# KohakuBlueleaf/UwUDiff

Measured on AMD Instinct MI355X. Metric: train images/sec (whole node), DiT-S/2 256^2 latent, higher is better.
Workload: dtype bf16; 1 GPU; DiT-S/2 (L12 D384 h6), 4x32x32 synthetic latents + pooled-text cond 1280, eps-MSE, AdamW lr1e-6 wd0.01 cosine; random-init weights; per_gpu_batch=768, global_batch=768, parallelism=dp1

## Files before the change

uwudiff_amd/csrc/attention_p256.hip:

```cpp
#include "common.h"

namespace {

constexpr int P_RING = 3;
template <int DH>
struct PGeom {
  static constexpr bool TAIL = DH > 64;
  static constexpr int SLOT = 16384 + (TAIL ? 2048 + 256 : 0);
  static constexpr int OFF_TT = 16384, OFF_TL = 16384 + 2048;
  static constexpr int OFF_DS = P_RING * SLOT;
  static constexpr int KIMG = 32768 + (TAIL ? 4096 : 0);
  static constexpr int OFF_K = OFF_DS + 32768;
  static constexpr int OFF_LSE = OFF_K + 2 * KIMG;
  static constexpr int OFF_DELTA = OFF_LSE + (TAIL ? 0 : 2 * 1024);
  static constexpr int OFF_ZERO = OFF_DELTA + 2 * 256;
  static constexpr int LDS = OFF_ZERO + (TAIL ? 16 : 0);
};
static_assert(PGeom<64>::LDS == 150016 && PGeom<72>::LDS <= 163840, "LDS budget");
constexpr int P_LDS = PGeom<64>::LDS;

struct PArgs {
  const bf16_t *q, *k, *v, *o, *dO;
  bf16_t *dq, *dk, *dv;
  const float* lse;
  int B, H, ldq, ldk, ldv, ldo, nheads;
  float scale;
};

__device__ __forceinline__ int fsw(int row) {
  return (((row >> 2) ^ (row >> 4)) & 1) | ((((row >> 3) ^ (row >> 4)) & 1) << 1) | (((row >> 1) & 1) << 2);
}
__device__ __forceinline__ int Fsw(int row) {
  return (row & 1) | (((row >> 2) & 1) << 1) | (((row >> 3) & 1) << 2) | (((row >> 1) & 1) << 3);
}

typedef short s16x4 __attribute__((ext_vector_type(4)));
typedef unsigned su32x2 __attribute__((ext_vector_type(2)));

__device__ __forceinline__ void glds16(const void* gsrc, unsigned lds_dst ) {
  unsigned keep;
  asm volatile("s_mov_b32 %0, m0\n\ts_mov_b32 m0, %2\n\ts_nop 0\n\tglobal_load_lds_dwordx4 %1, off\n\ts_mov_b32 m0, %0"
               : "=&s"(keep)
               : "v"(gsrc), "s"(lds_dst)
               : "memory");
}
__device__ __forceinline__ void glds4(const void* gsrc, unsigned lds_dst ) {
  unsigned keep;
  asm volatile("s_mov_b32 %0, m0\n\ts_mov_b32 m0, %2\n\ts_nop 0\n\tglobal_load_lds_dword %1, off\n\ts_mov_b32 m0, %0"
               : "=&s"(keep)
               : "v"(gsrc), "s"(lds_dst)
               : "memory");
}
__device__ __forceinline__ void glds16_s(const void* sbase , unsigned voff, unsigned lds_dst ) {
  unsigned keep;
  asm volatile("s_mov_b32 %0, m0\n\ts_mov_b32 m0, %3\n\ts_nop 0\n\tglobal_load_lds_dwordx4 %1, %2\n\ts_mov_b32 m0, %0"
               : "=&s"(keep)
               : "v"(voff), "s"(sbase), "s"(lds_dst)
               : "memory");
}
__device__ __forceinline__ f32x16 mfma32(const uint4& a, const uint4& b, f32x16 c) {
  return __builtin_amdgcn_mfma_f32_32x32x16_bf16(*reinterpret_cast<const bf16x8*>(&a), *reinterpret_cast<const bf16x8*>(&b), c, 0,
                                                 0, 0);
}
__device__ __forceinline__ f32x4 mfma16(const uint4& a, const uint4& b, f32x4 c) {
  return __builtin_amdgcn_mfma_f32_16x16x32_bf16(*reinterpret_cast<const bf16x8*>(&a), *reinterpret_cast<const bf16x8*>(&b), c, 0,
                                                 0, 0);
}
__device__ __forceinline__ uint4 pack8(const f32x16& x, int s) {
  bf16x8 f;
#pragma unroll
  for (int j = 0; j < 8; ++j) f[j] = (bf16_t)x[8 * s + j];
  return *reinterpret_cast<uint4*>(&f);
}

extern __shared__ __attribute__((aligned(16))) char p_smem[];

__device__ __forceinline__ void lane_halves(float x, float& lo, float& hi) {
  float a = x, b = x;
  asm volatile("v_nop\n\tv_nop\n\tv_permlane32_swap_b32 %0, %1" : "+v"(a), "+v"(b));
  lo = a;
  hi = b;
}

__device__ __forceinline__ uint4 tr_pair(unsigned a0, unsigned a1) {
  const s16x4 lo = __builtin_amdgcn_ds_read_tr16_b64_v4i16(
      (__attribute__((address_space(3))) s16x4*)((__attribute__((address_space(3))) char*)p_smem + a0));
  const s16x4 hi = __builtin_amdgcn_ds_read_tr16_b64_v4i16(
      (__attribute__((address_space(3))) s16x4*)((__attribute__((address_space(3))) char*)p_smem + a1));
  uint4 r;
  r.x = ((unsigned)(unsigned short)lo[0]) | ((unsigned)(unsigned short)lo[1] << 16);
  r.y = ((unsigned)(unsigned short)lo[2]) | ((unsigned)(unsigned short)lo[3] << 16);
  r.z = ((unsigned)(unsigned short)hi[0]) | ((unsigned)(unsigned short)hi[1] << 16);
  r.w = ((unsigned)(unsigned short)hi[2]) | ((unsigned)(unsigned short)hi[3] << 16);
  return r;
}

template <int DH>
__global__ void __launch_bounds__(512, 2) attn_bwd_p256(const PArgs a) {
  using G = PGeom<DH>;
  constexpr bool TAIL = G::TAIL;
  constexpr int T = 256, NKS = TAIL ? 5 : 4, NDT = TAIL ? 3 : 2;
  constexpr int P_SLOT = G::SLOT, P_OFF_DS = G::OFF_DS, P_OFF_K = G::OFF_K, P_OFF_LSE = G::OFF_LSE, P_OFF_DELTA = G::OFF_DELTA;
  constexpr int KIMG = G::KIMG;
  char* const smem = p_smem;
  const int tid = threadIdx.x, lane = tid & 63;
  const int wave = __builtin_amdgcn_readfirstlane(tid >> 6);
  const int r = lane & 31, h = lane >> 5;
  const int fr = lane & 15, fq = lane >> 4;
  const unsigned smem_base = (unsigned)(size_t)((const __attribute__((address_space(3))) char*)p_smem);
  const float c = a.scale * 1.4426950408889634f;
  const float ninv_scale = -1.f / a.scale;
  const int nmy = (a.nheads - (int)blockIdx.x + (int)gridDim.x - 1) / (int)gridDim.x;
  const int total = 4 * nmy;
  const int k0 = wave * 32;

  const int drow = tid >> 3;
  const int dchunk = (tid & 7) ^ fsw(drow);
  unsigned B0, A0, K0, D0, TQ0, TA0, KT0;
  auto phase1_consts = [&](int ln) {
    const int r_ = ln & 31, h_ = ln >> 5;
    B0 = (unsigned)(r_ * 128 + ((h_ ^ fsw(r_)) << 4));
    const int rowL = 4 * h_ + ((ln & 15) >> 2), chunkL = 2 * ((ln >> 4) & 1) + ((ln & 3) >> 1);
    A0 = (unsigned)(rowL * 128 + ((chunkL ^ fsw(rowL)) << 4) + 8 * (ln & 1));
    TQ0 = (unsigned)((r_ >> 3) * 256 + (r_ & 7) * 16);
    TA0 = (unsigned)(rowL * 16 + 8 * (ln & 1));
  };
  auto phase2_consts = [&](int ln) {
    const int fr_ = ln & 15, fq_ = ln >> 4;
    const int rowK = 8 * fq_ + (fr_ >> 2);
    K0 = (unsigned)(rowK * 128 + ((((fr_ & 3) >> 1) ^ fsw(rowK)) << 4) + 8 * (fr_ & 1));
    D0 = (unsigned)(rowK * 128 + (((fr_ & 3) ^ Fsw(rowK)) << 3));
    KT0 = (unsigned)(rowK * 16 + 8 * (fr_ & 1));
  };
  auto opaque_lane = [&]() {
    int ln = lane;
    asm volatile("" : "+v"(ln));
    return ln;
  };
  auto my_tid = [&]() {
    int x = tid;
    if constexpr (TAIL) asm volatile("" : "+v"(x));
    return x;
  };
  if constexpr (!TAIL) {
    phase1_consts(lane);
    phase2_consts(lane);
  }

  auto head_ptrs = [&](int j, int& b, int& hd) {
    const int bh = (int)blockIdx.x + j * (int)gridDim.x;
    b = bh / a.H;
    hd = bh - b * a.H;
  };
  uint4 oreg;
  unsigned otail = 0;
  auto issue_tile = [&](int g) {
    int b, hd;
    head_ptrs(g >> 2, b, hd);
    const int tid = my_tid(), lane = tid & 63, drow = tid >> 3, dchunk = (tid & 7) ^ fsw(drow);
    const int row = 64 * (g & 3) + drow;
    const bf16_t* qs = a.q + ((int64_t)b * T + row) * a.ldq + hd * DH + 8 * dchunk;
    const bf16_t* gs = a.dO + ((int64_t)b * T + row) * a.ldo + hd * DH + 8 * dchunk;
    const unsigned dst = smem_base + (unsigned)((g % P_RING) * P_SLOT + wave * 1024);
    glds16(qs, dst);
    glds16(gs, dst + 8192);
    oreg = *reinterpret_cast<const uint4*>(a.o + ((int64_t)b * T + row) * a.ldo + hd * DH + 8 * dchunk);
    if constexpr (TAIL) {
      const unsigned slot = smem_base + (unsigned)((g % P_RING) * P_SLOT);
      if (lane < 16) {
        const int64_t trow = (int64_t)b * T + 64 * (g & 3) + 8 * wave + (lane & 7);
        const bf16_t* src = lane < 8 ? a.q + trow * a.ldq + hd * DH + 64 : a.dO + trow * a.ldo + hd * DH + 64;
        glds16(src, slot + (unsigned)(G::OFF_TT + wave * 256));
      }
      glds4(a.lse + ((int64_t)b * a.H + hd) * T + 64 * (g & 3) + lane, slot + (unsigned)G::OFF_TL);
      otail = *reinterpret_cast<const unsigned*>(a.o + ((int64_t)b * T + row) * a.ldo + hd * DH + 64 + 2 * (tid & 3));
    }
  };
  auto issue_head = [&](int j) {
    int b, hd;
    head_ptrs(j, b, hd);
    const int tid = my_tid(), lane = tid & 63, drow = tid >> 3, dchunk = (tid & 7) ^ fsw(drow);
    const unsigned dst = smem_base + (unsigned)(P_OFF_K + (j & 1) * KIMG + wave * 1024);
#pragma unroll
    for (int p = 0; p < 4; ++p)
      glds16(a.k + ((int64_t)b * T + 64 * p + drow) * a.ldk + hd * DH + 8 * dchunk, dst + p * 8192);
    if constexpr (TAIL) {
      if (lane < 32)
        glds16(a.k + ((int64_t)b * T + 32 * wave + lane) * a.ldk + hd * DH + 64,
               smem_base + (unsigned)(P_OFF_K + (j & 1) * KIMG + 32768 + wave * 512));
    } else {
      glds4(a.lse + ((int64_t)b * a.H + hd) * T + 64 * (wave & 3) + lane,
            smem_base + (unsigned)(P_OFF_LSE + (j & 1) * 1024 + (wave & 3) * 256));
    }
  };
  uint4 kf[NKS], vf[NKS];
  auto load_kv = [&](int j) {
    int b, hd;
    head_ptrs(j, b, hd);
    const int tid = my_tid(), r = tid & 31, h = (tid >> 5) & 1;
#pragma unroll
    for (int s = 0; s < 4; ++s) {
      kf[s] = *reinterpret_cast<const uint4*>(a.k + ((int64_t)b * T + k0 + r) * a.ldk + hd * DH + 16 * s + 8 * h);
      vf[s] = *reinterpret_cast<const uint4*>(a.v + ((int64_t)b * T + k0 + r) * a.ldv + hd * DH + 16 * s + 8 * h);
    }
    if constexpr (TAIL) {
      kf[4] = *reinterpret_cast<const uint4*>(a.k + ((int64_t)b * T + k0 + r) * a.ldk + hd * DH + 64);
      vf[4] = *reinterpret_cast<const uint4*>(a.v + ((int64_t)b * T + k0 + r) * a.ldv + hd * DH + 64);
    }
  };
  auto delta_of = [&](int g) {
    const uint4 gch = *reinterpret_cast<const uint4*>(smem + (g % P_RING) * P_SLOT + 8192 + 16 * tid);
    const bf16x8 gv = *reinterpret_cast<const bf16x8*>(&gch), ov = *reinterpret_cast<const bf16x8*>(&oreg);
    float ds = 0.f;
#pragma unroll
    for (int e = 0; e < 8; ++e) ds += (float)gv[e] * (float)ov[e];
    if constexpr (TAIL) {
      const unsigned gtc = *reinterpret_cast<const unsigned*>(smem + (g % P_RING) * P_SLOT + G::OFF_TT + (drow >> 3) * 256 + 128 +
                                                              (drow & 7) * 16 + 4 * (tid & 3));
      const bf16x2 gt2 = *reinterpret_cast<const bf16x2*>(&gtc), ot2 = *reinterpret_cast<const bf16x2*>(&otail);
      const float dt2 = (float)gt2[0] * (float)ot2[0] + (float)gt2[1] * (float)ot2[1];
      ds += (tid & 4) ? 0.f : dt2;
    }
    ds += __builtin_bit_cast(float, __builtin_amdgcn_update_dpp(0, __builtin_bit_cast(int, ds), 0xB1, 0xF, 0xF, true));
    ds += __builtin_bit_cast(float, __builtin_amdgcn_update_dpp(0, __builtin_bit_cast(int, ds), 0x4E, 0xF, 0xF, true));
    ds += __builtin_bit_cast(float, __builtin_amdgcn_update_dpp(0, __builtin_bit_cast(int, ds), 0x141, 0xF, 0xF, true));
    if ((tid & 7) == 0) reinterpret_cast<float*>(smem + P_OFF_DELTA + (g & 1) * 256)[drow] = -ds;
  };

  f32x16 dkT[2], dvT[2];
  f32x4 dkt = {0.f, 0.f, 0.f, 0.f}, dvt = {0.f, 0.f, 0.f, 0.f};
#pragma unroll
  for (int dt = 0; dt < 2; ++dt) dkT[dt] = dvT[dt] = f32x16{};

  auto store_dkdv = [&](int j) {
    int b, hd;
    head_ptrs(j, b, hd);
    const int tid = my_tid(), lane = tid & 63, r = tid & 31, h = (tid >> 5) & 1;
    char* mine = smem + P_OFF_K + (j & 1) * KIMG + wave * 4096;
    char* mine_t = smem + P_OFF_K + (j & 1) * KIMG + 32768 + wave * 512;
#pragma unroll
    for (int which = 0; which < 2; ++which) {
#pragma unroll
      for (int dt = 0; dt < 2; ++dt)
#pragma unroll
        for (int g4 = 0; g4 < 4; ++g4) {
          const int d0 = 32 * dt + 8 * g4 + 4 * h;
          const f32x16& x = which ? dvT[dt] : dkT[dt];
          const float sc = which ? 1.f : a.scale;
          store4(reinterpret_cast<bf16_t*>(mine + r * 128 + (((d0 >> 3) ^ (r & 7)) << 4) + 2 * (d0 & 7)),
                 f32x4{x[4 * g4] * sc, x[4 * g4 + 1] * sc, x[4 * g4 + 2] * sc, x[4 * g4 + 3] * sc});
        }
      bf16_t* dst = (which ? a.dv : a.dk) + (int64_t)b * T * (which ? a.ldv : a.ldk) + hd * DH;
      const int ld = which ? a.ldv : a.ldk;
#pragma unroll
      for (int p = 0; p < 4; ++p) {
        const int key = 8 * p + (lane >> 3), ch = lane & 7;
        const uint4 x = *reinterpret_cast<const uint4*>(mine + key * 128 + ((ch ^ (key & 7)) << 4));
        *reinterpret_cast<uint4*>(dst + (int64_t)(k0 + key) * ld + 8 * ch) = x;
      }
      if constexpr (TAIL) {
        const f32x4 x = which ? dvt : dkt;
        const float sc = which ? 1.f : a.scale;
        store4(reinterpret_cast<bf16_t*>(mine_t + r * 16 + 8 * h), f32x4{x[0] * sc, x[1] * sc, x[2] * sc, x[3] * sc});
        const uint4 xt = *reinterpret_cast<const uint4*>(mine_t + r * 16);
        *reinterpret_cast<uint4*>(dst + (int64_t)(k0 + r) * ld + 64) = xt;
      }
    }
#pragma unroll
    for (int dt = 0; dt < 2; ++dt) dkT[dt] = dvT[dt] = f32x16{};
    dkt = dvt = f32x4{0.f, 0.f, 0.f, 0.f};
  };

  if (total == 0) return;
  if constexpr (TAIL)
    if (tid < 4) reinterpret_cast<unsigned*>(smem + G::OFF_ZERO)[tid] = 0u;
  issue_head(0);
  issue_tile(0);
  load_kv(0);
  __builtin_amdgcn_s_waitcnt(0x0070);
  asm volatile("" ::: "memory");
  __builtin_amdgcn_s_barrier();
  delta_of(0);
  if (1 < total) issue_tile(1);
  __builtin_amdgcn_s_waitcnt(0x0070);
  for (int g = 0; g < total; ++g) {
    const int j = g >> 2, t = g & 3;
    __builtin_amdgcn_s_waitcnt(TAIL ? 0x0072 : 0x0071);
    asm volatile("" ::: "memory");
    __builtin_amdgcn_s_barrier();
    if (t == 0 && j > 0) store_dkdv(j - 1);
    if (g + 1 < total) delta_of(g + 1);
    if (g + 2 < total) {
      issue_tile(g + 2);
      if (((g + 2) & 3) == 0) issue_head((g + 2) >> 2);
    }
    if constexpr (TAIL) phase1_consts(opaque_lane());
    const unsigned Qs = (unsigned)((g % P_RING) * P_SLOT), Gs = Qs + 8192;
    const float* ls = TAIL ? reinterpret_cast<const float*>(smem + (g % P_RING) * P_SLOT + G::OFF_TL)
                           : reinterpret_cast<const float*>(smem + P_OFF_LSE + (j & 1) * 1024) + 64 * t;
    const float* dl = reinterpret_cast<const float*>(smem + P_OFF_DELTA + (g & 1) * 256);
    char* const dsimg = smem + P_OFF_DS;
#pragma unroll
    for (int sub = 0; sub < 2; ++sub) {
      f32x16 S, dP;
#pragma unroll
      for (int g4 = 0; g4 < 4; ++g4) {
        const f32x4 l4 = load4(ls + 32 * sub + 8 * g4 + 4 * h);
        const f32x4 d4 = load4(dl + 32 * sub + 8 * g4 + 4 * h);
#pragma unroll
        for (int e = 0; e < 4; ++e) {
          S[4 * g4 + e] = l4[e] * ninv_scale;
          dP[4 * g4 + e] = d4[e];
        }
      }
#pragma unroll
      for (int s = 0; s < 4; ++s) {
        const unsigned off = (B0 ^ (unsigned)(s << 5)) + 4096u * sub;
        const uint4 qa = *reinterpret_cast<const uint4*>(smem + Qs + off);
        const uint4 ga = *reinterpret_cast<const uint4*>(smem + Gs + off);
        S = mfma32(qa, kf[s], S);
        dP = mfma32(ga, vf[s], dP);
      }
      if constexpr (TAIL) {
        const unsigned off = Qs + (unsigned)G::OFF_TT + TQ0 + 1024u * sub;
        const uint4 qa = *reinterpret_cast<const uint4*>(smem + (h ? (unsigned)G::OFF_ZERO : off));
        const uint4 ga = *reinterpret_cast<const uint4*>(smem + (h ? (unsigned)G::OFF_ZERO : off + 128));
        S = mfma32(qa, kf[4], S);
        dP = mfma32(ga, vf[4], dP);
      }
#pragma unroll
      for (int i = 0; i < 16; ++i) {
        const float p = __builtin_amdgcn_exp2f(S[i] * c);
        S[i] = p;
        dP[i] *= p;
      }
      bf16x2 dsp[8];
#pragma unroll
      for (int jj = 0; jj < 8; ++jj) dsp[jj] = bf16x2{(bf16_t)dP[2 * jj], (bf16_t)dP[2 * jj + 1]};
#pragma unroll
      for (int g4 = 0; g4 < 4; ++g4) {
        uint2 w;
        w.x = *reinterpret_cast<const unsigned*>(&dsp[2 * g4]);
        w.y = *reinterpret_cast<const unsigned*>(&dsp[2 * g4 + 1]);
        const int key = k0 + r;
        *reinterpret_cast<uint2*>(dsimg + key * 128 + (((8 * sub + 2 * g4 + h) ^ Fsw(key)) << 3)) = w;
      }
      f32x16 tv = {}, tk = {};
#pragma unroll
      for (int s2 = 0; s2 < 2; ++s2) {
        const uint4 pf = pack8(S, s2);
        uint4 dsf;
        dsf.x = *reinterpret_cast<const unsigned*>(&dsp[4 * s2]);
        dsf.y = *reinterpret_cast<const unsigned*>(&dsp[4 * s2 + 1]);
        dsf.z = *reinterpret_cast<const unsigned*>(&dsp[4 * s2 + 2]);
        dsf.w = *reinterpret_cast<const unsigned*>(&dsp[4 * s2 + 3]);
#pragma unroll
        for (int dt = 0; dt < 2; ++dt) {
          const unsigned x0 = (A0 ^ (unsigned)(0x30 * s2) ^ (unsigned)(0x40 * dt)) + 2048u * s2 + 4096u * sub;
          const unsigned x1 = (x0 ^ 0x20u) + 1024u;
          const uint4 gt = tr_pair(Gs + x0, Gs + x1);
          const uint4 qt = tr_pair(Qs + x0, Qs + x1);
          dvT[dt] = mfma32(gt, pf, dvT[dt]);
          dkT[dt] = mfma32(qt, dsf, dkT[dt]);
        }
        if constexpr (TAIL) {
          const unsigned x0 = Qs + (unsigned)G::OFF_TT + TA0 + 512u * s2 + 1024u * sub;
          const uint4 gt = tr_pair(x0 + 128u, x0 + 128u + 256u);
          const uint4 qt = tr_pair(x0, x0 + 256u);
          tv = mfma32(gt, pf, tv);
          tk = mfma32(qt, dsf, tk);
        }
      }
      if constexpr (TAIL) {
#pragma unroll
        for (int e = 0; e < 4; ++e) {
          dvt[e] += tv[e];
          dkt[e] += tk[e];
        }
      }
    }
    if (t == 3 && j + 1 < nmy) load_kv(j + 1);
    asm volatile("s_waitcnt lgkmcnt(0)" ::: "memory");
    __builtin_amdgcn_s_barrier();
    if constexpr (TAIL) phase2_consts(opaque_lane());
    const int qblk = wave & 3, db0 = 2 * (wave >> 2);
    const unsigned Ki = (unsigned)(P_OFF_K + (j & 1) * KIMG), Di = (unsigned)P_OFF_DS;
    const unsigned ka = K0 ^ (unsigned)(db0 << 5), kb = K0 ^ (unsigned)((db0 + 1) << 5), da = D0 ^ (unsigned)(qblk << 5);
    f32x4 acc0 = {0.f, 0.f, 0.f, 0.f}, acc1 = {0.f, 0.f, 0.f, 0.f}, acc2 = {0.f, 0.f, 0.f, 0.f};
#pragma unroll
    for (int kk = 0; kk < 8; ++kk) {
      const unsigned ko = 4096u * kk;
      const uint4 fa = tr_pair(Ki + ka + ko, Ki + (ka ^ 0x10u) + 512u + ko);
      const uint4 fb = tr_pair(Ki + kb + ko, Ki + (kb ^ 0x10u) + 512u + ko);
      const uint4 fd = tr_pair(Di + da + ko, Di + (da ^ 0x10u) + 512u + ko);
      acc0 = mfma16(fa, fd, acc0);
      acc1 = mfma16(fb, fd, acc1);
      if constexpr (TAIL) {
        const unsigned kt = Ki + 32768u + KT0 + 512u * kk;
        acc2 = mfma16(tr_pair(kt, kt + 64u), fd, acc2);
      }
    }
    int b, hd;
    head_ptrs(j, b, hd);
    const f32x4 v0 = acc0 * a.scale, v1 = acc1 * a.scale;
    const bf16x4 p0b = {(bf16_t)v0[0], (bf16_t)v0[1], (bf16_t)v0[2], (bf16_t)v0[3]};
    const bf16x4 p1b = {(bf16_t)v1[0], (bf16_t)v1[1], (bf16_t)v1[2], (bf16_t)v1[3]};
    const uint2 p0 = *reinterpret_cast<const uint2*>(&p0b), p1 = *reinterpret_cast<const uint2*>(&p1b);
    const su32x2 sx = __builtin_amdgcn_permlane16_swap(p0.x, p1.x, false, false);
    const su32x2 sy = __builtin_amdgcn_permlane16_swap(p0.y, p1.y, false, false);
    const bool odd = fq & 1;
    const int d = odd ? 16 * (db0 + 1) + 4 * (fq - 1) : 16 * db0 + 4 * fq;
    bf16_t* dst = a.dq + ((int64_t)b * T + 64 * t + 16 * qblk + fr) * a.ldq + hd * DH + d;
    *reinterpret_cast<uint4*>(dst) = uint4{sx[0], sy[0], sx[1], sy[1]};
    if constexpr (TAIL) {
      const f32x4 v2 = acc2 * a.scale;
      store4(a.dq + ((int64_t)b * T + 64 * t + 16 * qblk + fr) * a.ldq + hd * DH + 64 + 4 * (fq & 1), v2);
    }
  }
  asm volatile("s_waitcnt lgkmcnt(0)" ::: "memory");
  __builtin_amdgcn_s_barrier();
  store_dkdv(nmy - 1);
}

template <int DH>
struct FGeom {
  static constexpr bool TAIL = DH > 64;
  static constexpr int RING = TAIL ? 4 : 5;
  static constexpr int SLOT = 16384 + (TAIL ? 2048 : 0);
  static constexpr int OFF_TT = 16384;
  static constexpr int OST = 4096 + (TAIL ? 512 : 0);
  static constexpr int OFF_O = RING * SLOT;
  static constexpr int OFF_Q = OFF_O + 8 * OST;
  static constexpr int OFF_ZERO = OFF_Q + 32768 + (TAIL ? 4096 : 0);
  static constexpr int LDS = OFF_ZERO + (TAIL ? 16 : 0);
};
static_assert(FGeom<64>::LDS == 147456 && FGeom<72>::LDS <= 163840, "LDS budget");
constexpr int F_LDS = FGeom<64>::LDS;

struct FArgs {
  const bf16_t *q, *k, *v;
  bf16_t* out;
  float* lse;
  int B, H, ldq, ldk, ldv, ldo, nheads;
  float scale;
};

template <int N>
__device__ __forceinline__ void wait_vm_n() {
  asm volatile("s_waitcnt vmcnt(%0)" ::"n"(N) : "memory");
}
__device__ __forceinline__ void wait_vm(int n) {
  switch (n < 20 ? n : 20) {
    case 20: wait_vm_n<20>(); break;
    case 19: wait_vm_n<19>(); break;
    case 18: wait_vm_n<18>(); break;
    case 17: wait_vm_n<17>(); break;
    case 16: wait_vm_n<16>(); break;
    case 15: wait_vm_n<15>(); break;
    case 14: wait_vm_n<14>(); break;
    case 13: wait_vm_n<13>(); break;
    case 12: wait_vm_n<12>(); break;
    case 11: wait_vm_n<11>(); break;
    case 10: wait_vm_n<10>(); break;
    case 9: wait_vm_n<9>(); break;
    case 8: wait_vm_n<8>(); break;
    case 7: wait_vm_n<7>(); break;
    case 6: wait_vm_n<6>(); break;
    case 5: wait_vm_n<5>(); break;
    case 4: wait_vm_n<4>(); break;
    case 3: wait_vm_n<3>(); break;
    case 2: wait_vm_n<2>(); break;
    case 1: wait_vm_n<1>(); break;
    default: wait_vm_n<0>();
  }
}

template <int DH>
__global__ void __launch_bounds__(512, 2) attn_fwd_p256(const FArgs a) {
  using G = FGeom<DH>;
  constexpr bool TAIL = G::TAIL;
  constexpr int T = 256, NKS = TAIL ? 5 : 4, NDT = TAIL ? 3 : 2;
  constexpr int F_RING = G::RING, AHEAD = F_RING - 1, F_SLOT = G::SLOT, F_OFF_O = G::OFF_O, F_OFF_Q = G::OFF_Q;
  constexpr int TILE_OPS = TAIL ? 3 : 2, Q_OPS = TAIL ? 5 : 4, ST_OPS = TAIL ? 6 : 5;
  char* const smem = p_smem;
  const int tid = threadIdx.x, lane = tid & 63;
  const int wave = __builtin_amdgcn_readfirstlane(tid >> 6);
  const int r = lane & 31, h = lane >> 5;
  const unsigned smem_base = (unsigned)(size_t)((const __attribute__((address_space(3))) char*)p_smem);
  const float c = a.scale * 1.4426950408889634f;
  const int nmy = (a.nheads - (int)blockIdx.x + (int)gridDim.x - 1) / (int)gridDim.x;
  const int total = 4 * nmy;
  const int q0 = wave * 32;
  const int drow = tid >> 3;
  const int dchunk = (tid & 7) ^ fsw(drow);
  const unsigned B0 = (unsigned)(r * 128 + ((h ^ fsw(r)) << 4));
  const unsigned QR0 = (unsigned)(F_OFF_Q + (q0 + r) * 128 + ((h ^ fsw(q0 + r)) << 4));
  const int rowL = 4 * h + ((lane & 15) >> 2), chunkL = 2 * ((lane >> 4) & 1) + ((lane & 3) >> 1);
  const unsigned A0 = (unsigned)(rowL * 128 + ((chunkL ^ fsw(rowL)) << 4) + 8 * (lane & 1));
  const unsigned TQ0 = (unsigned)((r >> 3) * 256 + (r & 7) * 16);
  const unsigned TA0 = (unsigned)(rowL * 16 + 8 * (lane & 1));
  auto head_ptrs = [&](int j, int& b, int& hd) {
    const int bh = (int)blockIdx.x + j * (int)gridDim.x;
    b = bh / a.H;
    hd = bh - b * a.H;
  };
  const unsigned kvoff = (unsigned)((drow * a.ldk + 8 * dchunk) * 2), vvoff = (unsigned)((drow * a.ldv + 8 * dchunk) * 2);
  const unsigned qvoff = (unsigned)((drow * a.ldq + 8 * dchunk) * 2);
  const bf16_t *kb_n = nullptr, *vb_n = nullptr, *qb_n = nullptr;
  int b_c = 0, hd_c = 0;
  auto set_issue_head = [&](int j) {
    int b, hd;
    head_ptrs(j, b, hd);
    kb_n = a.k + (int64_t)b * T * a.ldk + hd * DH;
    vb_n = a.v + (int64_t)b * T * a.ldv + hd * DH;
    qb_n = a.q + (int64_t)b * T * a.ldq + hd * DH;
  };
  auto issue_tile = [&](int g) {
    const int t64 = 64 * (g & 3);
    const unsigned dst = smem_base + (unsigned)((g % F_RING) * F_SLOT + wave * 1024);
    glds16_s(kb_n, kvoff + (unsigned)(t64 * a.ldk * 2), dst);
    glds16_s(vb_n, vvoff + (unsigned)(t64 * a.ldv * 2), dst + 8192);
    if constexpr (TAIL) {
      if (lane < 16) {
        const int trow = t64 + 8 * wave + (lane & 7);
        const bf16_t* src = lane < 8 ? kb_n + (int64_t)trow * a.ldk + 64 : vb_n + (int64_t)trow * a.ldv + 64;
        glds16(src, smem_base + (unsigned)((g % F_RING) * F_SLOT + G::OFF_TT + wave * 256));
      }
    }
  };
  auto issue_q = [&]() {
#pragma unroll
    for (int p = 0; p < 4; ++p)
      glds16_s(qb_n, qvoff + (unsigned)(64 * p * a.ldq * 2), smem_base + (unsigned)(F_OFF_Q + p * 8192 + wave * 1024));
    if constexpr (TAIL) {
      if (lane < 32) glds16(qb_n + (int64_t)(32 * wave + lane) * a.ldq + 64, smem_base + (unsigned)(F_OFF_Q + 32768 + wave * 512));
    }
  };
  auto extras = [&](int i) { return ((i & 3) == 1 && (i >> 2) + 1 < nmy ? Q_OPS : 0) + ((i & 3) == 3 ? ST_OPS : 0); };
  auto younger = [&](int g) {
    int y = 0;
    const int gi = g - (F_RING - 1);
    if (gi < 0) {
      for (int x = g + 1; x < F_RING - 1; ++x) y += x < total ? TILE_OPS : 0;
    } else {
      y += extras(gi);
    }
    for (int i = gi < 0 ? 0 : gi + 1; i < g; ++i) y += (i + F_RING - 1 < total ? TILE_OPS : 0) + extras(i);
    return y;
  };
  if (total == 0) return;
  static_assert(AHEAD == 4 || AHEAD == 3, "the tile issued in iteration g belongs to the next head from t = 4 - AHEAD on");
  if constexpr (TAIL)
    if (tid < 4) reinterpret_cast<unsigned*>(smem + G::OFF_ZERO)[tid] = 0u;
  set_issue_head(0);
  head_ptrs(0, b_c, hd_c);
  issue_q();
#pragma unroll
  for (int g = 0; g < F_RING - 1; ++g) issue_tile(g);

  uint4 qf[NKS];
  f32x16 o[NDT];
  float m = -INFINITY, l = 0.f;
  for (int g = 0; g < total; ++g) {
    const int j = g >> 2, t = g & 3;
    int n_fly = younger(g);
    if (t == 0 && j > 0) {
      const int yq = (g - 2 + F_RING - 1 < total ? TILE_OPS : 0) + (g - 1 + F_RING - 1 < total ? TILE_OPS : 0) + ST_OPS;
      n_fly = yq < n_fly ? yq : n_fly;
    }
    wait_vm(n_fly);
    __builtin_amdgcn_s_barrier();
    if (t == 0) head_ptrs(j, b_c, hd_c);
    if (t == 4 - AHEAD && j + 1 < nmy) set_issue_head(j + 1);
    if (g + F_RING - 1 < total) issue_tile(g + F_RING - 1);
    if (t == 0) {
#pragma unroll
      for (int s = 0; s < 4; ++s) qf[s] = *reinterpret_cast<const uint4*>(smem + (QR0 ^ (unsigned)(s << 5)));
      if constexpr (TAIL)
        qf[4] = *reinterpret_cast<const uint4*>(smem + (h ? (unsigned)G::OFF_ZERO : (unsigned)(F_OFF_Q + 32768 + (q0 + r) * 16)));
#pragma unroll
      for (int dt = 0; dt < NDT; ++dt) o[dt] = f32x16{};
      m = -INFINITY;
      l = 0.f;
    }
    if (t == 1 && j + 1 < nmy) issue_q();
    const unsigned Ks = (unsigned)((g % F_RING) * F_SLOT), Vs = Ks + 8192;
    f32x16 s[2];
#pragma unroll
    for (int kt = 0; kt < 2; ++kt) {
      s[kt] = f32x16{};
#pragma unroll
      for (int ss = 0; ss < 4; ++ss) {
        const uint4 kfr = *reinterpret_cast<const uint4*>(smem + Ks + (B0 ^ (unsigned)(ss << 5)) + 4096u * kt);
        s[kt] = mfma32(kfr, qf[ss], s[kt]);
      }
      if constexpr (TAIL) {
        const uint4 kfr = *reinterpret_cast<const uint4*>(smem + Ks + (unsigned)G::OFF_TT + TQ0 + 1024u * kt);
        s[kt] = mfma32(kfr, qf[4], s[kt]);
      }
    }
    float mx = s[0][0];
#pragma unroll
    for (int kt = 0; kt < 2; ++kt)
#pragma unroll
      for (int i = 0; i < 16; ++i) mx = fmaxf(mx, s[kt][i]);
    {
      float lo, hi;
      lane_halves(mx, lo, hi);
      mx = fmaxf(lo, hi);
    }
    const float mn = fmaxf(m, mx);
    const float alpha = __builtin_amdgcn_exp2f((m - mn) * c);
    const float mc = mn * c;
    float ls = 0.f;
#pragma unroll
    for (int kt = 0; kt < 2; ++kt)
#pragma unroll
      for (int i = 0; i < 16; ++i) {
        const float p = __builtin_amdgcn_exp2f(s[kt][i] * c - mc);
        s[kt][i] = p;
        ls += p;
      }
    l = l * alpha + ls;
    m = mn;
#pragma unroll
    for (int dt = 0; dt < 2; ++dt)
#pragma unroll
      for (int i = 0; i < 16; ++i) o[dt][i] *= alpha;
    if constexpr (TAIL) {
#pragma unroll
      for (int i = 0; i < 4; ++i) o[2][i] *= alpha;
    }
#pragma unroll
    for (int kt = 0; kt < 2; ++kt)
#pragma unroll
      for (int s2 = 0; s2 < 2; ++s2) {
        const uint4 pf = pack8(s[kt], s2);
#pragma unroll
        for (int dt = 0; dt < 2; ++dt) {
          const unsigned x0 = (A0 ^ (unsigned)(0x30 * s2) ^ (unsigned)(0x40 * dt)) + 2048u * s2 + 4096u * kt;
          const uint4 vt = tr_pair(Vs + x0, Vs + (x0 ^ 0x20u) + 1024u);
          o[dt] = mfma32(vt, pf, o[dt]);
        }
        if constexpr (TAIL) {
          const unsigned x0 = Ks + (unsigned)G::OFF_TT + 128u + TA0 + 512u * s2 + 1024u * kt;
          o[2] = mfma32(tr_pair(x0, x0 + 256u), pf, o[2]);
        }
      }
    if (t == 3) {
      const int b = b_c, hd = hd_c;
      float lt;
      {
        float lo, hi;
        lane_halves(l, lo, hi);
        lt = lo + hi;
      }
      const float inv = 1.f / lt;
      char* mine = smem + F_OFF_O + wave * G::OST;
#pragma unroll
      for (int dt = 0; dt < 2; ++dt)
#pragma unroll
        for (int g4 = 0; g4 < 4; ++g4) {
          const int d0 = 32 * dt + 8 * g4 + 4 * h;
          store4(reinterpret_cast<bf16_t*>(mine + r * 128 + (((d0 >> 3) ^ (r & 7)) << 4) + 2 * (d0 & 7)),
                 f32x4{o[dt][4 * g4] * inv, o[dt][4 * g4 + 1] * inv, o[dt][4 * g4 + 2] * inv, o[dt][4 * g4 + 3] * inv});
        }
      bf16_t* ob = a.out + ((int64_t)b * T + q0) * a.ldo + hd * DH;
#pragma unroll
      for (int p = 0; p < 4; ++p) {
        const int row = 8 * p + (lane >> 3), ch = lane & 7;
        const uint4 x = *reinterpret_cast<const uint4*>(mine + row * 128 + ((ch ^ (row & 7)) << 4));
        *reinterpret_cast<uint4*>(ob + (int64_t)row * a.ldo + 8 * ch) = x;
      }
      if constexpr (TAIL) {
        store4(reinterpret_cast<bf16_t*>(mine + 4096 + r * 16 + 8 * h), f32x4{o[2][0] * inv, o[2][1] * inv, o[2][2] * inv, o[2][3] * inv});
        const uint4 xt = *reinterpret_cast<const uint4*>(mine + 4096 + r * 16);
        *reinterpret_cast<uint4*>(ob + (int64_t)r * a.ldo + 64) = xt;
      }
      a.lse[((int64_t)b * a.H + hd) * T + q0 + r] = m * a.scale + __logf(lt);
    }
  }
}

}

bool uwu_attn_p256_ok(int T, int Tk, int d, int ldq, int ldk, int ldv, int ldo) {
  static UwuEnv on("UWU_ATTN_P256");
  if (on.get().is('0') || T != 256 || Tk != 256 || ldq % 8 || ldk % 8 || ldv % 8 || ldo % 8 || uwu_dev_cus() <= 0) return false;
  if (d == 64) return uwu_dev_lds_fits(P_LDS);
  static UwuEnv on72("UWU_ATTN_P256_D72");
  return d == 72 && !on72.get().is('0') && uwu_dev_lds_fits(PGeom<72>::LDS);
}

int uwu_attn_p256_bwd(const void* q, const void* k, const void* v, const void* o, const void* dO, const float* lse, void* dq,
                      void* dk, void* dv, int B, int H, int d, int ldq, int ldk, int ldv, int ldo, float scale, hipStream_t st) {
  static unsigned char done[UWU_MAX_DEV];
  const int n_cu = uwu_dev_cus();
  if (d == 72) {
    static unsigned char done72[UWU_MAX_DEV];
    if (n_cu <= 0 || !uwu_func_lds(reinterpret_cast<const void*>(attn_bwd_p256<72>), PGeom<72>::LDS, done72)) {
      uwu_set_error("attention_bwd(p256, d = 72): the device cannot give a workgroup %d bytes of LDS", (int)PGeom<72>::LDS);
      return UWU_ELAUNCH;
    }
    PArgs a{};
    a.q = (const bf16_t*)q; a.k = (const bf16_t*)k; a.v = (const bf16_t*)v; a.o = (const bf16_t*)o; a.dO = (const bf16_t*)dO;
    a.dq = (bf16_t*)dq; a.dk = (bf16_t*)dk; a.dv = (bf16_t*)dv; a.lse = lse;
    a.B = B; a.H = H; a.ldq = ldq; a.ldk = ldk; a.ldv = ldv; a.ldo = ldo; a.nheads = B * H; a.scale = scale;
    const int grid = a.nheads < n_cu ? a.nheads : n_cu;
    hipLaunchKernelGGL(attn_bwd_p256<72>, dim3(grid), dim3(512), PGeom<72>::LDS, st, a);
    UWU_LAUNCH_CHECK("attention_bwd(p256, d = 72)");
    return UWU_OK;
  }
  if (n_cu <= 0 || !uwu_func_lds(reinterpret_cast<const void*>(attn_bwd_p256<64>), P_LDS, done)) {
    uwu_set_error("attention_bwd(p256): the device cannot give a workgroup %d bytes of LDS", (int)P_LDS);
    return UWU_ELAUNCH;
  }
  PArgs a{};
  a.q = (const bf16_t*)q; a.k = (const bf16_t*)k; a.v = (const bf16_t*)v; a.o = (const bf16_t*)o; a.dO = (const bf16_t*)dO;
  a.dq = (bf16_t*)dq; a.dk = (bf16_t*)dk; a.dv = (bf16_t*)dv; a.lse = lse;
  a.B = B; a.H = H; a.ldq = ldq; a.ldk = ldk; a.ldv = ldv; a.ldo = ldo; a.nheads = B * H; a.scale = scale;
  const int grid = a.nheads < n_cu ? a.nheads : n_cu;
  hipLaunchKernelGGL(attn_bwd_p256<64>, dim3(grid), dim3(512), P_LDS, st, a);
  UWU_LAUNCH_CHECK("attention_bwd(p256)");
  return UWU_OK;
}

bool uwu_attn_p256_fwd_ok(int nheads, int T, int Tk, int d, int ldq, int ldk, int ldv, int ldo) {
  static UwuEnv on("UWU_ATTN_P256F");
  if (on.get().is('0')) return false;
  if (!on.is('1') && nheads < 1024) return false;
  if (T != 256 || Tk != 256 || ldq % 8 || ldk % 8 || ldv % 8 || ldo % 8 || uwu_dev_cus() <= 0) return false;
  if (d == 64) return uwu_dev_lds_fits(F_LDS);
  static UwuEnv on72("UWU_ATTN_P256F_D72");
  return d == 72 && !on72.get().is('0') && uwu_dev_lds_fits(FGeom<72>::LDS);
}

int uwu_attn_p256_fwd(const void* q, const void* k, const void* v, void* o, float* lse, int B, int H, int d, int ldq, int ldk, int ldv,
                      int ldo, float scale, hipStream_t st) {
  static unsigned char done[2][UWU_MAX_DEV];
  const int n_cu = uwu_dev_cus();
  const int lds = d == 72 ? FGeom<72>::LDS : F_LDS;
  const void* fn = d == 72 ? reinterpret_cast<const void*>(attn_fwd_p256<72>) : reinterpret_cast<const void*>(attn_fwd_p256<64>);
  if (n_cu <= 0 || !uwu_func_lds(fn, lds, done[d == 72])) {
    uwu_set_error("attention_fwd(p256): the device cannot give a workgroup %d bytes of LDS", lds);
    return UWU_ELAUNCH;
  }
  FArgs a{};
  a.q = (const bf16_t*)q; a.k = (const bf16_t*)k; a.v = (const bf16_t*)v; a.out = (bf16_t*)o; a.lse = lse;
  a.B = B; a.H = H; a.ldq = ldq; a.ldk = ldk; a.ldv = ldv; a.ldo = ldo; a.nheads = B * H; a.scale = scale;
  const int grid = a.nheads < n_cu ? a.nheads : n_cu;
  if (d == 72) hipLaunchKernelGGL(attn_fwd_p256<72>, dim3(grid), dim3(512), lds, st, a);
  else hipLaunchKernelGGL(attn_fwd_p256<64>, dim3(grid), dim3(512), lds, st, a);
  UWU_LAUNCH_CHECK("attention_fwd(p256)");
  return UWU_OK;
}
```

Before: 17490 images/s.

## Use scalar-base global loads and counted vmcnt waits in attention backward

Rewrites the attention backward kernel's global loads to use SGPR base pointers with 32-bit VGPR offsets, computed once per head, replacing per-load 64-bit address arithmetic. K fragments are now read from the already-staged LDS K image instead of being fetched from global memory again, and only V is loaded from global. The blanket vmcnt(0)-style waits become precise counted waits based on the number of outstanding ops per stage. The dkdv store is moved after the next tile's issue so loads and stores overlap. The hand-counted wait thresholds are fragile: if an op count is wrong, data can be read before it lands.

```diff
diff --git a/uwudiff_amd/csrc/attention_p256.hip b/uwudiff_amd/csrc/attention_p256.hip
--- a/uwudiff_amd/csrc/attention_p256.hip
+++ b/uwudiff_amd/csrc/attention_p256.hip
@@ -57,6 +57,30 @@
                : "=&s"(keep)
                : "v"(voff), "s"(sbase), "s"(lds_dst)
                : "memory");
+}
+typedef unsigned u32x4 __attribute__((ext_vector_type(4)));
+__device__ __forceinline__ u32x4 gload16_s(const void* sbase , unsigned voff) {
+  u32x4 x;
+  asm volatile("global_load_dwordx4 %0, %1, %2" : "=v"(x) : "v"(voff), "s"(sbase) : "memory");
+  return x;
+}
+__device__ __forceinline__ unsigned gload4_s(const void* sbase , unsigned voff) {
+  unsigned x;
+  asm volatile("global_load_dword %0, %1, %2" : "=v"(x) : "v"(voff), "s"(sbase) : "memory");
+  return x;
+}
+__device__ __forceinline__ void landed(u32x4& x) { asm volatile("" : "+v"(x)); }
+__device__ __forceinline__ void landed(unsigned& x) { asm volatile("" : "+v"(x)); }
+template <int N>
+__device__ __forceinline__ void wait_vm_n() {
+  asm volatile("s_waitcnt vmcnt(%0)" ::"n"(N) : "memory");
+}
+template <int N>
+__device__ __forceinline__ void wait_vm_lgkm0() {
+  asm volatile("s_waitcnt vmcnt(%0) lgkmcnt(0)" ::"n"(N) : "memory");
+}
+__device__ __forceinline__ f32x16 mfma32(const uint4& a, const u32x4& b, f32x16 c) {
+  return __builtin_amdgcn_mfma_f32_32x32x16_bf16(*reinterpret_cast<const bf16x8*>(&a), __builtin_bit_cast(bf16x8, b), c, 0, 0, 0);
 }
 __device__ __forceinline__ f32x16 mfma32(const uint4& a, const uint4& b, f32x16 c) {
   return __builtin_amdgcn_mfma_f32_32x32x16_bf16(*reinterpret_cast<const bf16x8*>(&a), *reinterpret_cast<const bf16x8*>(&b), c, 0,
@@ -152,65 +176,75 @@
     b = bh / a.H;
     hd = bh - b * a.H;
   };
-  uint4 oreg;
+  constexpr int TILE_OPS = TAIL ? 6 : 3, HEAD_OPS = 5, ST_OPS = TAIL ? 10 : 8, V_OPS = NKS, DQ_OPS = TAIL ? 2 : 1;
+  u32x4 oreg;
   unsigned otail = 0;
+  const bf16_t *qb_n = nullptr, *gb_n = nullptr, *ob_n = nullptr, *kb_n = nullptr, *vb_n = nullptr;
+  const float* lb_n = nullptr;
+  bf16_t* dqb_c = nullptr;
+  auto set_issue_head = [&](int j) {
+    int b, hd;
+    head_ptrs(j, b, hd);
+    qb_n = a.q + (int64_t)b * T * a.ldq + hd * DH;
+    gb_n = a.dO + (int64_t)b * T * a.ldo + hd * DH;
+    ob_n = a.o + (int64_t)b * T * a.ldo + hd * DH;
+    kb_n = a.k + (int64_t)b * T * a.ldk + hd * DH;
+    vb_n = a.v + (int64_t)b * T * a.ldv + hd * DH;
+    lb_n = a.lse + ((int64_t)b * a.H + hd) * T;
+  };
   auto issue_tile = [&](int g) {
-    int b, hd;
-    head_ptrs(g >> 2, b, hd);
     const int tid = my_tid(), lane = tid & 63, drow = tid >> 3, dchunk = (tid & 7) ^ fsw(drow);
-    const int row = 64 * (g & 3) + drow;
-    const bf16_t* qs = a.q + ((int64_t)b * T + row) * a.ldq + hd * DH + 8 * dchunk;
-    const bf16_t* gs = a.dO + ((int64_t)b * T + row) * a.ldo + hd * DH + 8 * dchunk;
+    const int t64 = 64 * (g & 3);
+    const unsigned qv = (unsigned)((drow * a.ldq + 8 * dchunk) * 2), gv = (unsigned)((drow * a.ldo + 8 * dchunk) * 2);
     const unsigned dst = smem_base + (unsigned)((g % P_RING) * P_SLOT + wave * 1024);
-    glds16(qs, dst);
-    glds16(gs, dst + 8192);
-    oreg = *reinterpret_cast<const uint4*>(a.o + ((int64_t)b * T + row) * a.ldo + hd * DH + 8 * dchunk);
+    glds16_s(qb_n + (int64_t)t64 * a.ldq, qv, dst);
+    glds16_s(gb_n + (int64_t)t64 * a.ldo, gv, dst + 8192);
+    oreg = gload16_s(ob_n + (int64_t)t64 * a.ldo, gv);
     if constexpr (TAIL) {
       const unsigned slot = smem_base + (unsigned)((g % P_RING) * P_SLOT);
       if (lane < 16) {
-        const int64_t trow = (int64_t)b * T + 64 * (g & 3) + 8 * wave + (lane & 7);
-        const bf16_t* src = lane < 8 ? a.q + trow * a.ldq + hd * DH + 64 : a.dO + trow * a.ldo + hd * DH + 64;
+        const int trow = t64 + 8 * wave + (lane & 7);
+        const bf16_t* src = lane < 8 ? qb_n + (int64_t)trow * a.ldq + 64 : gb_n + (int64_t)trow * a.ldo + 64;
         glds16(src, slot + (unsigned)(G::OFF_TT + wave * 256));
       }
-      glds4(a.lse + ((int64_t)b * a.H + hd) * T + 64 * (g & 3) + lane, slot + (unsigned)G::OFF_TL);
-      otail = *reinterpret_cast<const unsigned*>(a.o + ((int64_t)b * T + row) * a.ldo + hd * DH + 64 + 2 * (tid & 3));
+      glds4(lb_n + t64 + lane, slot + (unsigned)G::OFF_TL);
+      otail = gload4_s(ob_n + (int64_t)t64 * a.ldo, (unsigned)((drow * a.ldo + 64 + 2 * (tid & 3)) * 2));
     }
   };
   auto issue_head = [&](int j) {
-    int b, hd;
-    head_ptrs(j, b, hd);
     const int tid = my_tid(), lane = tid & 63, drow = tid >> 3, dchunk = (tid & 7) ^ fsw(drow);
+    const unsigned kv = (unsigned)((drow * a.ldk + 8 * dchunk) * 2);
     const unsigned dst = smem_base + (unsigned)(P_OFF_K + (j & 1) * KIMG + wave * 1024);
 #pragma unroll
     for (int p = 0; p < 4; ++p)
-      glds16(a.k + ((int64_t)b * T + 64 * p + drow) * a.ldk + hd * DH + 8 * dchunk, dst + p * 8192);
+      glds16_s(kb_n + (int64_t)(64 * p) * a.ldk, kv, dst + p * 8192);
     if constexpr (TAIL) {
       if (lane < 32)
-        glds16(a.k + ((int64_t)b * T + 32 * wave + lane) * a.ldk + hd * DH + 64,
-               smem_base + (unsigned)(P_OFF_K + (j & 1) * KIMG + 32768 + wave * 512));
+        glds16(kb_n + (int64_t)(32 * wave + lane) * a.ldk + 64, smem_base + (unsigned)(P_OFF_K + (j & 1) * KIMG + 32768 + wave * 512));
     } else {
-      glds4(a.lse + ((int64_t)b * a.H + hd) * T + 64 * (wave & 3) + lane,
-            smem_base + (unsigned)(P_OFF_LSE + (j & 1) * 1024 + (wave & 3) * 256));
-    }
-  };
-  uint4 kf[NKS], vf[NKS];
-  auto load_kv = [&](int j) {
-    int b, hd;
-    head_ptrs(j, b, hd);
+      glds4(lb_n + 64 * (wave & 3) + lane, smem_base + (unsigned)(P_OFF_LSE + (j & 1) * 1024 + (wave & 3) * 256));
+    }
+  };
+  uint4 kf[NKS];
+  u32x4 vf[NKS];
+  auto load_v = [&]() {
     const int tid = my_tid(), r = tid & 31, h = (tid >> 5) & 1;
-#pragma unroll
-    for (int s = 0; s < 4; ++s) {
-      kf[s] = *reinterpret_cast<const uint4*>(a.k + ((int64_t)b * T + k0 + r) * a.ldk + hd * DH + 16 * s + 8 * h);
-      vf[s] = *reinterpret_cast<const uint4*>(a.v + ((int64_t)b * T + k0 + r) * a.ldv + hd * DH + 16 * s + 8 * h);
-    }
-    if constexpr (TAIL) {
-      kf[4] = *reinterpret_cast<const uint4*>(a.k + ((int64_t)b * T + k0 + r) * a.ldk + hd * DH + 64);
-      vf[4] = *reinterpret_cast<const uint4*>(a.v + ((int64_t)b * T + k0 + r) * a.ldv + hd * DH + 64);
-    }
+    const bf16_t* vb = vb_n + (int64_t)k0 * a.ldv;
+    const unsigned vv = (unsigned)((r * a.ldv + 8 * h) * 2);
+#pragma unroll
+    for (int s = 0; s < 4; ++s) vf[s] = gload16_s(vb, vv + 32u * s);
+    if constexpr (TAIL) vf[4] = gload16_s(vb, (unsigned)((r * a.ldv + 64) * 2));
+  };
+  auto read_kf = [&](int j) {
+    if constexpr (TAIL) phase1_consts(opaque_lane());
+    const unsigned Ki = (unsigned)(P_OFF_K + (j & 1) * KIMG);
+#pragma unroll
+    for (int s = 0; s < 4; ++s) kf[s] = *reinterpret_cast<const uint4*>(smem + Ki + (unsigned)(k0 * 128) + (B0 ^ (unsigned)(s << 5)));
+    if constexpr (TAIL) kf[4] = *reinterpret_cast<const uint4*>(smem + Ki + 32768u + (unsigned)((k0 + (my_tid() & 31)) * 16));
   };
   auto delta_of = [&](int g) {
     const uint4 gch = *reinterpret_cast<const uint4*>(smem + (g % P_RING) * P_SLOT + 8192 + 16 * tid);
-    const bf16x8 gv = *reinterpret_cast<const bf16x8*>(&gch), ov = *reinterpret_cast<const bf16x8*>(&oreg);
+    const bf16x8 gv = *reinterpret_cast<const bf16x8*>(&gch), ov = __builtin_bit_cast(bf16x8, oreg);
     float ds = 0.f;
 #pragma unroll
     for (int e = 0; e < 8; ++e) ds += (float)gv[e] * (float)ov[e];
@@ -274,25 +308,44 @@
   if (total == 0) return;
   if constexpr (TAIL)
     if (tid < 4) reinterpret_cast<unsigned*>(smem + G::OFF_ZERO)[tid] = 0u;
+  set_issue_head(0);
   issue_head(0);
   issue_tile(0);
-  load_kv(0);
-  __builtin_amdgcn_s_waitcnt(0x0070);
-  asm volatile("" ::: "memory");
+  load_v();
+  wait_vm_lgkm0<0>();
+  landed(oreg);
+  landed(otail);
+#pragma unroll
+  for (int s = 0; s < NKS; ++s) landed(vf[s]);
   __builtin_amdgcn_s_barrier();
+  read_kf(0);
   delta_of(0);
   if (1 < total) issue_tile(1);
-  __builtin_amdgcn_s_waitcnt(0x0070);
+  wait_vm_lgkm0<0>();
   for (int g = 0; g < total; ++g) {
     const int j = g >> 2, t = g & 3;
-    __builtin_amdgcn_s_waitcnt(TAIL ? 0x0072 : 0x0071);
-    asm volatile("" ::: "memory");
+    if (t == 1 && j > 0) wait_vm_lgkm0<DQ_OPS + ST_OPS>();
+    else if (t == 0 && j > 0) wait_vm_lgkm0<DQ_OPS + V_OPS>();
+    else wait_vm_lgkm0<DQ_OPS>();
+    landed(oreg);
+    if constexpr (TAIL) landed(otail);
     __builtin_amdgcn_s_barrier();
-    if (t == 0 && j > 0) store_dkdv(j - 1);
+    if (t == 0) {
+      int b, hd;
+      head_ptrs(j, b, hd);
+      dqb_c = a.dq + (int64_t)b * T * a.ldq + hd * DH;
+    }
     if (g + 1 < total) delta_of(g + 1);
     if (g + 2 < total) {
+      if (t == 2) set_issue_head(j + 1);
       issue_tile(g + 2);
-      if (((g + 2) & 3) == 0) issue_head((g + 2) >> 2);
+      if (t == 2) issue_head(j + 1);
+    }
+    if (t == 0 && j > 0) {
+      store_dkdv(j - 1);
+      wait_vm_n<DQ_OPS + TILE_OPS + ST_OPS>();
+#pragma unroll
+      for (int s = 0; s < NKS; ++s) landed(vf[s]);
     }
     if constexpr (TAIL) phase1_consts(opaque_lane());
     const unsigned Qs = (unsigned)((g % P_RING) * P_SLOT), Gs = Qs + 8192;
@@ -379,7 +432,10 @@
         }
       }
     }
-    if (t == 3 && j + 1 < nmy) load_kv(j + 1);
+    if (t == 3 && j + 1 < nmy) {
+      load_v();
+      read_kf(j + 1);
+    }
     asm volatile("s_waitcnt lgkmcnt(0)" ::: "memory");
     __builtin_amdgcn_s_barrier();
     if constexpr (TAIL) phase2_consts(opaque_lane());
@@ -400,8 +456,6 @@
         acc2 = mfma16(tr_pair(kt, kt + 64u), fd, acc2);
       }
     }
-    int b, hd;
-    head_ptrs(j, b, hd);
     const f32x4 v0 = acc0 * a.scale, v1 = acc1 * a.scale;
     const bf16x4 p0b = {(bf16_t)v0[0], (bf16_t)v0[1], (bf16_t)v0[2], (bf16_t)v0[3]};
     const bf16x4 p1b = {(bf16_t)v1[0], (bf16_t)v1[1], (bf16_t)v1[2], (bf16_t)v1[3]};
@@ -410,11 +464,11 @@
     const su32x2 sy = __builtin_amdgcn_permlane16_swap(p0.y, p1.y, false, false);
     const bool odd = fq & 1;
     const int d = odd ? 16 * (db0 + 1) + 4 * (fq - 1) : 16 * db0 + 4 * fq;
-    bf16_t* dst = a.dq + ((int64_t)b * T + 64 * t + 16 * qblk + fr) * a.ldq + hd * DH + d;
-    *reinterpret_cast<uint4*>(dst) = uint4{sx[0], sy[0], sx[1], sy[1]};
+    bf16_t* const dqt = dqb_c + (int64_t)(64 * t + 16 * qblk) * a.ldq;
+    *reinterpret_cast<uint4*>(reinterpret_cast<char*>(dqt) + (unsigned)((fr * a.ldq + d) * 2)) = uint4{sx[0], sy[0], sx[1], sy[1]};
     if constexpr (TAIL) {
       const f32x4 v2 = acc2 * a.scale;
-      store4(a.dq + ((int64_t)b * T + 64 * t + 16 * qblk + fr) * a.ldq + hd * DH + 64 + 4 * (fq & 1), v2);
+      store4(reinterpret_cast<bf16_t*>(reinterpret_cast<char*>(dqt) + (unsigned)((fr * a.ldq + 64 + 4 * (fq & 1)) * 2)), v2);
     }
   }
   asm volatile("s_waitcnt lgkmcnt(0)" ::: "memory");
@@ -445,10 +499,6 @@
   float scale;
 };
 
-template <int N>
-__device__ __forceinline__ void wait_vm_n() {
-  asm volatile("s_waitcnt vmcnt(%0)" ::"n"(N) : "memory");
-}
 __device__ __forceinline__ void wait_vm(int n) {
   switch (n < 20 ? n : 20) {
     case 20: wait_vm_n<20>(); break;
```

After: 17580 images/s, median of 6. About the same (+0.5%).
